# librosa/librosa

Hardware: AMD Instinct MI355X
Metric: STFT+mel frames/sec (n_fft=2048 hop=512) (higher is better)
Workload: dtype f32

## Files before the change

### librosa_amd/csrc/lra_kernels.h

```cpp
#pragma once

#ifndef LRA_ABLATE
#define LRA_ABLATE 0
#endif

#include <cmath>
#include <limits>

#include "lra_fft.h"

#if defined(LRA_PHASE_TIMER) && !defined(LRA_HOSTSIM)
__device__ unsigned long long lra_phase_ticks[16];
#define LRA_TICK(i)                                                    \
    do {                                                               \
        const unsigned long long now__ = __builtin_amdgcn_s_memtime(); \
        tick_acc[i] += now__ - tick_prev;                              \
        tick_prev = now__;                                             \
    } while (0)
#define LRA_TICK_DECL unsigned long long tick_acc[16] = {}, tick_prev = __builtin_amdgcn_s_memtime()
#define LRA_TICK_FLUSH                                                                    \
    do {                                                                                  \
        if ((threadIdx.x & 63) == 0)                                                      \
            for (int i__ = 0; i__ < 16; ++i__) atomicAdd(&lra_phase_ticks[i__], tick_acc[i__]); \
    } while (0)
// ... 676 lines not shown

template <class Cfg> LRA_HD void mel2_combine(const StftArgs<typename Cfg::real>& a, int clip, int frame, int tf, int it, int tile, Lds sh, Lds psum, Lds stage) {
    using T = typename Cfg::real;
    using C = typename Cfg::cplx;
    constexpr int NB = Cfg::M + 1;
#if LRA_ABLATE == 15
    if (a.n_mels != 12345) return;
#endif
    for (int m = tf; m < a.n_mels; m += Cfg::TF) {
        constexpr int UNR = 6;
        int first[2], cnt[2];
        LRA_UNROLL
        for (int h = 0; h < 2; ++h) {
            const int d = lds_ld<int>(sh, NB * (int)sizeof(C) + (Cfg::TF + m + h) * (int)sizeof(int));
            first[h] = d & 0xfff;
            cnt[h] = d >> 12;
        }
        T x[2][UNR];
        LRA_UNROLL
        for (int h = 0; h < 2; ++h) {
            LRA_UNROLL
            for (int q = 0; q < UNR; ++q) {
                const bool ok = q < cnt[h];
                x[h][q] = lds_ld<T>(psum, ((ok ? first[h] + q : 0) * 2 + (1 - h)) * (int)sizeof(T));
                if (!ok) x[h][q] = (T)0;
            }
        }
        T part[2];
        LRA_UNROLL
        for (int h = 0; h < 2; ++h) {
            T acc = (T)0;
            LRA_UNROLL
            for (int q = 0; q < UNR; ++q) acc += x[h][q];
            for (int q = UNR; q < cnt[h]; ++q) acc += lds_ld<T>(psum, ((first[h] + q) * 2 + (1 - h)) * (int)sizeof(T));
            part[h] = acc;
        }
        const T v = part[0] + part[1];
        if (tile == 1) a.Mel[((long long)clip * a.n_mels + m) * a.n_frames + frame] = v;
        else lds_st<T>(stage, (m * tile + (it % tile)) * (int)sizeof(T), v);
    }
}

constexpr int MELR_PMAX = 16;
template <class Cfg> LRA_HD int melr_w_slot(int i) { return i + 2 * (i / (Cfg::R / 2)); }
template <class Cfg> LRA_HD int melr_keep_off() { return ((melr_w_slot<Cfg>(Cfg::M) + 1) * 2 * (int)sizeof(typename Cfg::real) + 15) / 16 * 16; }
template <class Cfg> LRA_HD int melr_addr_off() { return melr_keep_off<Cfg>(); }
constexpr int MELR_PHOIST_N = 4;
template <class Cfg> LRA_HD bool melr_needs_table(int n_mels, int pmax) { return pmax > melr_ph<Cfg>() || n_mels > melr_nb<Cfg>() * Cfg::TF; }
template <class Cfg> LRA_HD int melr_shared_bytes(int n_mels, int pmax) {
    return ((melr_addr_off<Cfg>() + (melr_needs_table<Cfg>(n_mels, pmax) ? n_mels * 2 * pmax * (int)sizeof(int) : 0) + 15) / 16) * 16;
}
template <class Cfg> constexpr bool melr_fits() {
    return Cfg::R == 16 && (1 << Cfg::PADSHIFT) % (Cfg::R / 2) == 0 && (Cfg::R * Cfg::TF + 2) * 2 * (int)sizeof(typename Cfg::real) <= Cfg::FRAME_BYTES;
}

template <class Cfg> LRA_HD void melr_tables_to_lds(const StftArgs<typename Cfg::real>& a, int tid, Lds sh) {
    using T = typename Cfg::real;
    using C = typename Cfg::cplx;
    const C* __restrict__ w2 = reinterpret_cast<const C*>(a.melr_w);
    for (int k = tid; k < Cfg::M + 1; k += Cfg::NT) lds_st<C>(sh, melr_w_slot<Cfg>(k) * (int)sizeof(C), w2[k]);
    if (melr_needs_table<Cfg>(a.n_mels, a.melr_pmax))
        for (int i = tid; i < a.n_mels * 2 * a.melr_pmax; i += Cfg::NT) lds_st<int>(sh, melr_addr_off<Cfg>() + i * (int)sizeof(int), a.melr_addr[i]);
}

template <class Cfg> LRA_HD void split_read_runs(FftRegs<Cfg>& rg, Lds fr, int tf) {
    using C = typename Cfg::cplx;
    constexpr int BPL = Cfg::R / 2, M = Cfg::M;
    const int ba = Cfg::phys(BPL * tf) * (int)sizeof(C);
    const int bm = Cfg::phys(M - BPL * tf - 1) * (int)sizeof(C);
    const int b0 = Cfg::phys((M - BPL * tf) & (M - 1)) * (int)sizeof(C);
    LRA_UNROLL
    for (int j = 0; j < BPL; ++j) {
        rg.v[2 * j] = lds_ld<C>(fr, ba + j * (int)sizeof(C));
        rg.v[2 * j + 1] = lds_ld<C>(fr, j == 0 ? b0 : bm - (j - 1) * (int)sizeof(C));
    }
    if (tf == 0) rg.mid = lds_ld<C>(fr, Cfg::phys(M / 2) * (int)sizeof(C));
}

template <class Cfg, int PM> LRA_HD void melr_split_accumulate(const StftArgs<typename Cfg::real>& a, bool valid, int tf, FftRegs<Cfg>& rg, Lds rs, Lds sh) {
    using T = typename Cfg::real;
    using C = typename Cfg::cplx;
    constexpr int BPL = Cfg::R / 2, M = Cfg::M, TF = Cfg::TF;
    C ab[2 * BPL];
    LRA_UNROLL
    for (int j = 0; j < BPL; ++j) {
        const int k = BPL * tf + j;
        C xk, xm;
        if (k == 0) {
            const C z0 = rg.v[0];
            xk = mk<T>((T)2 * (z0.x + z0.y), (T)0);
            xm = mk<T>((T)2 * (z0.x - z0.y), (T)0);
            if (valid && a.nonfinite_flag && !(std::fabs(xk.x) <= std::numeric_limits<T>::max())) LRA_ATOMIC_OR(a.nonfinite_flag, 1u);
        } else {
            split_pair<T>(rg.v[2 * j], rg.v[2 * j + 1], Cfg::HOIST ? rg.twr[j] : a.twr[k], xk, xm);
        }
        const T pk = spec_power<T, PM>(xk, a.power), pm = spec_power<T, PM>(xm, a.power);
        const C wk = lds_ld<C>(sh, ((BPL + 2) * tf + j) * (int)sizeof(C)), wm = lds_ld<C>(sh, ((BPL + 2) * (TF + tf) + j) * (int)sizeof(C));
        ab[j] = mk<T>(wk.x * pk, wk.y * pk);
        ab[BPL + j] = mk<T>(wm.x * pm, wm.y * pm);
    }
    LRA_UNROLL
    for (int run = 0; run < 2; ++run) {
        C acc = mk<T>((T)0, (T)0);
        LRA_UNROLL
        for (int j = 0; j < BPL; ++j) {
            const int jj = run * BPL + j;
            const T keep = rg.keep[jj];
            acc = mk<T>(acc.x * keep + ab[jj].x, acc.y * keep + ab[jj].y);
            lds_st<C>(rs, (jj * TF + tf) * (int)sizeof(C), acc);
        }
    }
    if (tf == 0) {
        const C xmid = mk<T>((T)2 * rg.mid.x, (T)-2 * rg.mid.y);
        const T pmid = spec_power<T, PM>(xmid, a.power);
        const C wq = lds_ld<C>(sh, melr_w_slot<Cfg>(M) * (int)sizeof(C));
        lds_st<C>(rs, a.melr_mid, mk<T>(wq.x * pmid, wq.y * pmid));
        lds_st<C>(rs, a.melr_zero, mk<T>((T)0, (T)0));
    }
}

#ifndef LRA_MEL_PAIR_READS
#define LRA_MEL_PAIR_READS 1
#endif
template <class Cfg, class RG> LRA_HD void melr_hoist(const StftArgs<typename Cfg::real>& a, int tf, RG& rg, int base = 0) {
    constexpr int PH = RG::MELR_PHOIST;
    LRA_UNROLL
    for (int jj = 0; jj < Cfg::R; ++jj) rg.keep[jj] = a.melr_keep[jj * Cfg::TF + tf];
    LRA_UNROLL
    for (int b = 0; b < RG::MELR_NB; ++b) {
        const int m = RG::MELR_NB * tf + b;
        LRA_UNROLL
        for (int h = 0; h < 2; ++h) {
            LRA_UNROLL
            for (int q = 0; q < PH; ++q) {
                const int ad = base + (m < a.n_mels ? a.melr_addr[(h * a.melr_pmax + q) * a.n_mels + m] : a.melr_zero);
                rg.mad[b][h * PH + q] = (LRA_MEL_PAIR_READS && sizeof(typename Cfg::real) == 4) ? (ad & ~(2 * (int)sizeof(typename Cfg::real) - 1)) : ad;
            }
        }
    }
}

#ifndef LRA_MEL_ALIGNED_BURSTS
#define LRA_MEL_ALIGNED_BURSTS 1
#endif
#ifndef LRA_MEL_BURST16
#define LRA_MEL_BURST16 1
#endif
template <class Cfg, class RG> LRA_HD int melr_tile_slot(const StftArgs<typename Cfg::real>& a, int clip, int frame, int it, int b, long long row0) {
    constexpr int MT = RG::MELR_TILE;
    if (!LRA_MEL_ALIGNED_BURSTS) return it & (MT - 1);
    if ((a.n_frames & 3) == 0 && Cfg::TF >= 64) return (int)(((long long)clip * a.n_mels * a.n_frames + (long long)b * a.n_frames + frame) & (MT - 1));
    return (int)((row0 + frame) & (MT - 1));
}
template <class Cfg, class RG> LRA_HD void melr_burst(const StftArgs<typename Cfg::real>& a, long long row0, int frame, int s8, int it, int b, RG& rg) {
    using T = typename Cfg::real;
    constexpr int MT = RG::MELR_TILE;
    T* __restrict__ row = a.Mel + (row0 + frame - s8);
    if constexpr (sizeof(T) == 4 && (MT == 8 || MT == 4)) {
        if (LRA_MEL_BURST16 && s8 == MT - 1 && it >= MT - 1) {
            store4_unaligned(row, rg.mt[b][0], rg.mt[b][1], rg.mt[b][2], rg.mt[b][3]);
            if constexpr (MT == 8) store4_unaligned(row + 4, rg.mt[b][4], rg.mt[b][5], rg.mt[b][6], rg.mt[b][7]);
            return;
        }
    }
    LRA_UNROLL
    for (int k = 0; k < MT; ++k)
        if (k <= s8 && k >= s8 - it) row[k] = rg.mt[b][k];
}

template <class Cfg, class RG> LRA_HD void melr_combine(const StftArgs<typename Cfg::real>& a, int clip, int frame, int tf, int it, int tile, bool last_of_slot, RG& rg, Lds sh,
                                                        Lds rs, Lds stage, Lds rs_hoisted) {
    using T = typename Cfg::real;
    constexpr int PH = RG::MELR_PHOIST, TF = Cfg::TF, NB = RG::MELR_NB;
    const bool more = a.melr_pmax > PH;
    constexpr int GB = NB * 2 * PH > 16 ? 16 / (2 * PH) : NB;
    T x[NB][2 * PH];
    LRA_UNROLL
    for (int b = 0; b < NB; ++b) {
      if (b % GB == 0) {
        LRA_UNROLL
        for (int bb = b; bb < b + GB; ++bb) {
            LRA_UNROLL
            for (int q = 0; q < 2 * PH; ++q) {
                if constexpr (LRA_MEL_PAIR_READS && sizeof(T) == 4) {
                    const cx<T> pr = lds_ld<cx<T>>(rs_hoisted, rg.mad[bb][q]);
                    x[bb][q] = q < PH ? pr.y : pr.x;
                } else {
                    x[bb][q] = lds_ld<T>(rs_hoisted, rg.mad[bb][q]);
                }
            }
        }
      }
        const int m = NB * tf + b;
        if (m >= a.n_mels) break;
        T part[2];
        LRA_UNROLL
        for (int h = 0; h < 2; ++h) {
            T acc = (T)0;
            LRA_UNROLL
            for (int q = 0; q < PH; ++q) acc += x[b][h * PH + q];
            if (LRA_UNLIKELY(more)) {
                for (int q = PH; q < a.melr_pmax; ++q)
                    acc += lds_ld<T>(rs, lds_ld<int>(sh, melr_addr_off<Cfg>() + ((h * a.melr_pmax + q) * a.n_mels + m) * (int)sizeof(int)));
            }
            part[h] = acc;
        }
        const T v = part[0] + part[1];
        if (tile == 1) {
            constexpr int MT = RG::MELR_TILE;
            const long long row0 = ((long long)clip * a.n_mels + m) * a.n_frames;
            const int s8 = melr_tile_slot<Cfg, RG>(a, clip, frame, it, b, row0);
            LRA_UNROLL
            for (int k = 0; k < MT; ++k) rg.mt[b][k] = k == s8 ? v : rg.mt[b][k];
            if (last_of_slot || s8 == MT - 1) melr_burst<Cfg, RG>(a, row0, frame, s8, it, b, rg);
        } else {
            lds_st<T>(stage, (m * tile + (it % tile)) * (int)sizeof(T), v);
        }
    }
    for (int m = tf + NB * TF; m < a.n_mels; m += TF) {
        T part[2];
        LRA_UNROLL
        for (int h = 0; h < 2; ++h) {
            T acc = (T)0;
            for (int q = 0; q < a.melr_pmax; ++q)
                acc += lds_ld<T>(rs, lds_ld<int>(sh, melr_addr_off<Cfg>() + ((h * a.melr_pmax + q) * a.n_mels + m) * (int)sizeof(int)));
            part[h] = acc;
        }
        const T v = part[0] + part[1];
        if (tile == 1) a.Mel[((long long)clip * a.n_mels + m) * a.n_frames + frame] = v;
        else lds_st<T>(stage, (m * tile + (it % tile)) * (int)sizeof(T), v);
    }
}

#define LRA_MID_PASS(Cfg, p, rg, lds, tw, slot_bytes) LRA_MID_PASS_TO(Cfg, Cfg::P, p, rg, lds, tw, slot_bytes)
#define LRA_MID_PASS_TO(Cfg, END, p, rg, lds, tw, slot_bytes)                                             \
    if (END > p) {                                                                                        \
        LRA_PHASE(Cfg::NT, tid) {                                                                         \
            pass_read<Cfg, (p < Cfg::P ? p : 0)>(LRA_R(rg).v, lds_sub(lds, (slot_of<Cfg>(tid)) * (slot_bytes)), lane_of<Cfg>(tid)); \
        } LRA_PHASE_END_SYNC(Cfg::WAVE_SYNC)                                                              \
        LRA_TICK(2 * p);                                                                                  \
        LRA_PHASE(Cfg::NT, tid) {                                                                         \
            pass_dft<Cfg, (p < Cfg::P ? p : 0)>(LRA_R(rg), lane_of<Cfg>(tid), tw);                          \
            pass_write<Cfg, (p < Cfg::P ? p : 0)>(LRA_R(rg).v, lds_sub(lds, (slot_of<Cfg>(tid)) * (slot_bytes)), lane_of<Cfg>(tid)); \
        } LRA_PHASE_END_SYNC(Cfg::WAVE_SYNC)                                                              \
        LRA_TICK(2 * p + 1);                                                                              \
    }

template <class Cfg> constexpr int stft_ring_off() { return Cfg::FRAME_BYTES; }
template <class Cfg> constexpr int stft_tile_off() { return Cfg::FRAME_BYTES + Cfg::N * (int)sizeof(typename Cfg::real); }
template <class Cfg> inline int stft_slot_bytes(int mode, int n_mels, int tile) {
    int b = stft_tile_off<Cfg>();
    if (mode == OUT_MEL || ((mode == OUT_MEL2 || mode == OUT_MELR) && tile > 1)) b += ((n_mels * tile * (int)sizeof(typename Cfg::real) + 15) / 16) * 16;
    if (mode == OUT_MEL2) b += mel2_psum_bytes<Cfg>(n_mels);
    return b;
}

template <class Cfg, int MODE, int PM = POW_TWO, int RAM = 0> LRA_HD void stft_block(const StftArgs<typename Cfg::real>& a_in, const int blk, Lds lds) {
    constexpr bool RA = RAM == 1, DIRECT = RAM >= 2;
    constexpr int RHD = 1 << (RAM >= 3 ? RAM - 2 : 0);
    static_assert(RAM <= 2 || RegRing<Cfg, RHD>::ok, "register ring: the hop must be a whole number of pass-0 rows");
    static_assert(!DIRECT || MODE == OUT_COMPLEX || MODE == OUT_POWER, "direct framing serves the complex / power epilogues");
    StftArgs<typename Cfg::real> a = a_in;
    const int clip = blk / a.wg_per_clip;
    const int f_first = (blk % a.wg_per_clip) * a.frames_per_wg;
    const int iters = a.frames_per_wg / Cfg::FPB;
    const int slot_bytes = a.slot_bytes;
    const int tile = a.mel_tile;
    constexpr bool DEFER = MODE == OUT_MEL2 && !(LRA_ABLATE >= 11 && LRA_ABLATE <= 13);
#ifndef LRA_MEL_LATE_PF
#define LRA_MEL_LATE_PF 1
#endif
    constexpr bool LATE_PF = DEFER && LRA_MEL_LATE_PF;
#ifndef LRA_PF_EARLY
#define LRA_PF_EARLY 1
#endif
    constexpr bool PF_EARLY = !LATE_PF && LRA_PF_EARLY;
#ifndef LRA_SPLIT_ONE_BARRIER
#define LRA_SPLIT_ONE_BARRIER 1
#endif
    constexpr bool SPLIT_NO_LDS = LRA_SPLIT_ONE_BARRIER && (MODE == OUT_COMPLEX || MODE == OUT_POWER);
#ifndef LRA_MIRROR32
#define LRA_MIRROR32 1
#endif
    constexpr bool MIRROR = LRA_MIRROR32 && (RAM == 3 || RAM == 6 || LRA_MIRROR32 > 1) && mirror32_cfg_ok<Cfg>();
    constexpr int MID_END = Cfg::P - (MIRROR ? 1 : 0);
    LRA_REGS(FftRegs<Cfg>, rg, Cfg::NT);
    LRA_PHASE(Cfg::NT, tid) {
        hoist_tables<Cfg>(LRA_R(rg), lane_of<Cfg>(tid), a.win, a.tw, a.twr, false, MODE == OUT_MELR);
        if (MIRROR) mirror32_hoist<Cfg>(LRA_R(rg), lane_of<Cfg>(tid), a.tw, a.twr);
        if (MODE == OUT_MEL2) mel2_tables_to_lds<Cfg>(a, tid, lds_sub(lds, a.shared_off));
        if (MODE == OUT_MELR) {
            melr_tables_to_lds<Cfg>(a, tid, lds_sub(lds, a.shared_off));
            melr_hoist<Cfg>(a, lane_of<Cfg>(tid), LRA_R(rg));
        }
    } LRA_PHASE_END_SYNC(Cfg::WAVE_SYNC && MODE != OUT_MEL2 && MODE != OUT_MELR)
    LRA_PHASE(Cfg::NT, tid) {
        const int slot = slot_of<Cfg>(tid), tf = lane_of<Cfg>(tid);
        if (RHD > 1 || DIRECT) {
            LRA_UNROLL
            for (int e = 0; e < Cfg::R; ++e) LRA_R(rg).nxt[e] = mk<typename Cfg::real>((typename Cfg::real)0, (typename Cfg::real)0);
        }
        if (RHD > 1) {
            regring_fill<Cfg, RHD>(a, clip, f_first + slot * iters, tf, LRA_R(rg));
        } else if (DIRECT) {
            stft_direct_fetch<Cfg>(a, clip, f_first + slot * iters, tf, LRA_R(rg));
        } else {
            stft_ring_fill<Cfg>(a, clip, f_first + slot * iters, tf, lds_sub(lds, slot * slot_bytes + stft_ring_off<Cfg>()));
            if (PF_EARLY && iters > 1) stft_ring_prefetch<Cfg, RA>(a, clip, f_first + slot * iters + 1, tf, LRA_R(rg));
        }
    } LRA_PHASE_END_SYNC(Cfg::WAVE_SYNC)
    int done = 0;
    LRA_TICK_DECL;
    for (int it = 0; it < iters; ++it) {
        if (f_first + it >= a.n_frames) break;
        LRA_TICK(0);
        if (!Cfg::HOIST) { LRA_LAUNDER(a.win); LRA_LAUNDER(a.tw); LRA_LAUNDER(a.twr); }
        if (MODE == OUT_MELR) lra_setprio<LRA_V1_PRIO_A>();
        else if (MODE == OUT_COMPLEX || MODE == OUT_POWER) lra_setprio<LRA_V1_PRIO_CA>();
        LRA_PHASE(Cfg::NT, tid) {
            const int slot = slot_of<Cfg>(tid), tf = lane_of<Cfg>(tid), frame = f_first + slot * iters + it;
// ... 828 lines not shown
```

### librosa_amd/csrc/lra_kernels_pc.h

```cpp
#pragma once

#include "lra_kernels2.h"

namespace lra {

#ifndef LRA_PC_PRIO_PA
#define LRA_PC_PRIO_PA 3
#endif
#ifndef LRA_PC_PRIO_PS
#define LRA_PC_PRIO_PS 2
#endif
#ifndef LRA_PC_PRIO_CA
#define LRA_PC_PRIO_CA 0
#endif
#ifndef LRA_PC_PRIO_CB
#define LRA_PC_PRIO_CB 1
#endif
#ifndef LRA_PC_ROTATE
#define LRA_PC_ROTATE 1
#endif
#ifndef LRA_PC_SPIN_LIMIT
#define LRA_PC_SPIN_LIMIT (1 << 22)
#endif

template <class Cfg> struct PcLayout {
    using T = typename Cfg::real;
    static constexpr int NP = 2;
    static constexpr int NT = (NP + 1) * Cfg::TF;
    static constexpr int FRAME = Cfg::FRAME_BYTES;
    static constexpr int PW = (v2_pw_bytes<Cfg>() + 15) / 16 * 16;
    static constexpr int RS = ((Cfg::R * (Cfg::TF + LRA_MEL_RS_PITCH_EXTRA) + 2) * 2 * (int)sizeof(T) + 15) / 16 * 16;
    static constexpr int frame_off(int s) { return s * FRAME; }
    static constexpr int pw_off(int s) { return NP * FRAME + s * PW; }
    static constexpr int rs_off() { return NP * (FRAME + PW); }
    static constexpr int flags_off() { return rs_off() + RS; }
    static constexpr int ready_off(int s) { return flags_off() + 4 * s; }
    static constexpr int consumed_off(int s) { return flags_off() + 4 * (NP + s); }
    static constexpr int BYTES = flags_off() + 16;
};

template <class Cfg> constexpr bool pc_cfg_ok() { return v23_cfg_ok<Cfg>() && Cfg::TF == 64 && v2_pw_swz<Cfg>() && melr_fits<Cfg>() && sizeof(typename Cfg::real) == 4; }
template <class Cfg> LRA_HD bool pc_bank_ok(int n_mels, int pmax) { return n_mels >= 1 && n_mels <= 2 * Cfg::TF && pmax <= 4; }

template <class Cfg> LRA_HD bool pc_fits_budget(int hd, int power_mode) {
    if (power_mode != POW_TWO && power_mode != POW_ONE) return false;
    if (hd == 8) return true;
    return hd == 4 && (power_mode == POW_TWO || Cfg::PLAN == 1);
}

template <class Cfg> struct PcRegs {
    using T = typename Cfg::real;
    using C = typename Cfg::cplx;
    static constexpr int NB = 2, PH = 4, TILE = 8, NP = PcLayout<Cfg>::NP;
    C w[Cfg::R];
    C wq;
    T keep[Cfg::R];
    T pw[Cfg::R], pw_extra;
    int mad[NB][2 * PH];
    T mt[NP][NB][TILE];
};
template <class Cfg> struct PcTile {
    static constexpr int MELR_TILE = PcRegs<Cfg>::TILE;
    typename Cfg::real (&mt)[PcRegs<Cfg>::NB][PcRegs<Cfg>::TILE];
};

#ifdef LRA_HOSTSIM
LRA_HD int pc_flag_load(Lds l, int off) { return lds_ld<int>(l, off); }
LRA_HD void pc_flag_store(Lds l, int off, int v) { lds_st<int>(l, off, v); }
LRA_HD void pc_wait(Lds, int, int, unsigned int*) {}
LRA_HD void pc_fence() {}
#else
__device__ __forceinline__ void pc_fence() {
    __builtin_amdgcn_fence(__ATOMIC_RELEASE, "wavefront");
    __builtin_amdgcn_wave_barrier();
    __builtin_amdgcn_fence(__ATOMIC_ACQUIRE, "wavefront");
}
__device__ __forceinline__ int pc_flag_load(Lds l, int off) { return *(const volatile __attribute__((address_space(3))) int*)(l.base + off); }
__device__ __forceinline__ void pc_flag_store(Lds l, int off, int v) { *(volatile __attribute__((address_space(3))) int*)(l.base + off) = v; }
__device__ __forceinline__ void pc_wait(Lds l, int off, int want, unsigned int* sticky) {
    int spins = 0;
    while (true) {
        const int v = LRA_UNIFORM(pc_flag_load(l, off));
        if (LRA_LIKELY(v >= want)) break;
        if (LRA_UNLIKELY(++spins > LRA_PC_SPIN_LIMIT)) {
            if (sticky && (threadIdx.x & 63) == 0) atomicOr(sticky, 2u);
            break;
        }
        __builtin_amdgcn_s_sleep(2);
    }
    pc_fence();
}
#endif

template <class Cfg, int HD> LRA_HD void pc_producer_prologue(const StftArgs<typename Cfg::real>& a, int clip, int frame0, int tf, Regs2<Cfg, HD>& rg) {
    using T = typename Cfg::real;
    if constexpr (Cfg::PLAN == 1) v3_hoist<Cfg, HD>(rg, tf, a.win, a.tw, a.twr);
    else v2_hoist<Cfg, HD>(rg, tf, a.win, a.tw, a.twr);
    v2_fill<Cfg, HD>(a, clip, frame0, tf, rg);
    if constexpr (v2_rotate_asm_ok<Cfg, HD>() && LRA_PC_ROTATE) {
        LRA_UNROLL
        for (int e = 0; e < Cfg::R; ++e) { LRA_KEEP(rg.raw[e].x); LRA_KEEP(rg.raw[e].y); }
    }
    LRA_UNROLL
    for (int e = 0; e < Regs2<Cfg, HD>::NEW; ++e) rg.pf[e] = mk<T>((T)0, (T)0);
}
template <class Cfg, int HD> LRA_HD void pc_producer_pass0(const StftArgs<typename Cfg::real>& a, int clip, int frame, int it, bool more, int tf, Regs2<Cfg, HD>& rg, Lds fr) {
    if (v2_rotate_asm_ok<Cfg, HD>() && LRA_PC_ROTATE) {
        v2_window_rotating<Cfg, HD>(it, rg);
        if (more) v2_issue_loads<Cfg, HD>(a, clip, frame + 1, tf, rg);
        v2_pass0_dft<Cfg, HD>(tf, rg, fr);
    } else {
        if (it > 0) v2_shift<Cfg, HD>(rg);
        if (more) v2_issue_loads<Cfg, HD>(a, clip, frame + 1, tf, rg);
        v2_pass0<Cfg, HD>(frame < a.n_frames, tf, rg, fr);
    }
}

template <class Cfg, int p> LRA_HD void pc_mid_dft_write(typename Cfg::cplx* v, const typename Cfg::cplx* treg, Lds fr, int tf) {
    if constexpr (Cfg::PLAN == 1) {
        v3_mid_twiddle_dft<Cfg>(v, treg);
        v3_mid_write<Cfg>(v, fr, tf);
    } else {
        pass_twiddle_dft_reg<Cfg, p>(v, treg);
        pass_write<Cfg, p>(v, fr, tf);
    }
}
template <class Cfg, int HD> LRA_HD void pc_last_read(Regs2<Cfg, HD>& rg, Lds fr, int tf) {
    if constexpr (Cfg::PLAN == 1) v3_last_read<Cfg, HD>(rg, fr, tf);
    else v2_last_read<Cfg, HD>(rg, fr, tf);
}
template <class Cfg, int HD, int PM> LRA_HD void pc_last_power_row(const StftArgs<typename Cfg::real>& a, int clip, int frame, int tf, Regs2<Cfg, HD>& rg, Lds pwr) {
    if constexpr (Cfg::PLAN == 1) v3_last_split_store<Cfg, HD, OUT_MELR, PM, false>(a, clip, frame, frame < a.n_frames, tf, rg, pwr);
    else v2_last_split_store<Cfg, HD, OUT_MELR, PM, false, false>(a, clip, frame, frame < a.n_frames, tf, rg, pwr);
}

template <class Cfg> LRA_HD void pc_consumer_prologue(const StftArgs<typename Cfg::real>& a, int tf, PcRegs<Cfg>& rg) {
    using T = typename Cfg::real;
    using C = typename Cfg::cplx;
    using RG = PcRegs<Cfg>;
    constexpr int BPL = Cfg::R / 2, TF = Cfg::TF;
    const C* __restrict__ w2 = reinterpret_cast<const C*>(a.melr_w);
    LRA_UNROLL
    for (int run = 0; run < 2; ++run) {
        LRA_UNROLL
        for (int j = 0; j < BPL; ++j) rg.w[run * BPL + j] = w2[BPL * (run * TF + tf) + j];
    }
    rg.wq = w2[Cfg::M];
    LRA_UNROLL
    for (int jj = 0; jj < Cfg::R; ++jj) rg.keep[jj] = a.melr_keep[jj * TF + tf];
    LRA_UNROLL
    for (int b = 0; b < RG::NB; ++b) {
        const int m = RG::NB * tf + b;
        LRA_UNROLL
        for (int h = 0; h < 2; ++h) {
            LRA_UNROLL
            for (int q = 0; q < RG::PH; ++q) {
                const int ad = PcLayout<Cfg>::rs_off() + (m < a.n_mels ? a.melr_addr[(h * a.melr_pmax + q) * a.n_mels + m] : a.melr_zero);
                rg.mad[b][h * RG::PH + q] = ad & ~(2 * (int)sizeof(T) - 1);
            }
        }
    }
    LRA_UNROLL
    for (int s = 0; s < RG::NP; ++s) {
        LRA_UNROLL
        for (int b = 0; b < RG::NB; ++b) {
            LRA_UNROLL
            for (int k = 0; k < RG::TILE; ++k) rg.mt[s][b][k] = (T)0;
        }
    }
    rg.pw_extra = (T)0;
}
template <class Cfg> LRA_HD void pc_runs_read(PcRegs<Cfg>& rg, Lds pwr, int tf) {
    using T = typename Cfg::real;
    constexpr int BPL = Cfg::R / 2;
    static_assert(BPL == 8, "runs of 8 bins");
    LRA_UNROLL
    for (int run = 0; run < 2; ++run) {
        const int first = 8 * (run * Cfg::TF + tf);
        const V4<T> lo = lds_ld<V4<T>>(pwr, v2_pw_index<Cfg>(first) * (int)sizeof(T)), hi = lds_ld<V4<T>>(pwr, v2_pw_index<Cfg>(first + 4) * (int)sizeof(T));
        T* d = rg.pw + run * BPL;
        d[0] = lo.a; d[1] = lo.b; d[2] = lo.c; d[3] = lo.d; d[4] = hi.a; d[5] = hi.b; d[6] = hi.c; d[7] = hi.d;
    }
    rg.pw_extra = lds_ld<T>(pwr, (tf == 0 ? v2_pw_index<Cfg>(Cfg::M) : 0) * (int)sizeof(T));
}
template <class Cfg> LRA_HD void pc_accumulate(const StftArgs<typename Cfg::real>& a, int tf, PcRegs<Cfg>& rg, Lds rs) {
    using T = typename Cfg::real;
    using C = typename Cfg::cplx;
    constexpr int BPL = Cfg::R / 2, TF = Cfg::TF;
    LRA_UNROLL
    for (int run = 0; run < 2; ++run) {
        C acc = mk<T>((T)0, (T)0);
        LRA_UNROLL
        for (int j = 0; j < BPL; ++j) {
            const int jj = run * BPL + j;
            const T p = rg.pw[jj], keep = rg.keep[jj];
            acc = mk<T>(acc.x * keep + rg.w[jj].x * p, acc.y * keep + rg.w[jj].y * p);
            lds_st<C>(rs, (jj * mel_runs_pitch(TF, 1) + tf) * (int)sizeof(C), acc);
        }
    }
    if (tf == 0) {
        lds_st<C>(rs, a.melr_mid, mk<T>(rg.wq.x * rg.pw_extra, rg.wq.y * rg.pw_extra));
        lds_st<C>(rs, a.melr_zero, mk<T>((T)0, (T)0));
    }
}
template <class Cfg, int S> LRA_HD void pc_combine(const StftArgs<typename Cfg::real>& a, int clip, int frame, int tf, int it, bool last_of_slot, PcRegs<Cfg>& rg, Lds wg) {
    using T = typename Cfg::real;
    using RG = PcRegs<Cfg>;
    constexpr int PH = RG::PH, NB = RG::NB, MT = RG::TILE;
    T x[NB][2 * PH];
    LRA_UNROLL
    for (int b = 0; b < NB; ++b) {
        LRA_UNROLL
        for (int q = 0; q < 2 * PH; ++q) {
            const cx<T> pr = lds_ld<cx<T>>(wg, rg.mad[b][q]);
            x[b][q] = q < PH ? pr.y : pr.x;
        }
    }
    PcTile<Cfg> tile{rg.mt[S]};
    LRA_UNROLL
    for (int b = 0; b < NB; ++b) {
        const int m = NB * tf + b;
        if (m >= a.n_mels) break;
        T part[2];
        LRA_UNROLL
        for (int h = 0; h < 2; ++h) {
            T acc = (T)0;
            LRA_UNROLL
            for (int q = 0; q < PH; ++q) acc += x[b][h * PH + q];
            part[h] = acc;
        }
        const T v = part[0] + part[1];
        const long long row0 = ((long long)clip * a.n_mels + m) * a.n_frames;
        const int s8 = melr_tile_slot<Cfg, PcTile<Cfg>>(a, clip, frame, it, b, row0);
        LRA_UNROLL
        for (int k = 0; k < MT; ++k) rg.mt[S][b][k] = k == s8 ? v : rg.mt[S][b][k];
        if (last_of_slot || s8 == MT - 1) melr_burst<Cfg, PcTile<Cfg>>(a, row0, frame, s8, it, b, tile);
    }
}

template <class Cfg, int HD, int PM = POW_TWO> LRA_HD void stft_pc_block(const StftArgs<typename Cfg::real>& a_in, const int blk, Lds lds) {
    static_assert(pc_cfg_ok<Cfg>(), "producer / consumer mel kernel: one wave per frame, mirrored last pass, swizzled power row");
    using T = typename Cfg::real;
    using L = PcLayout<Cfg>;
    using RG = Regs2<Cfg, HD>;
    constexpr int NP = L::NP, TF = Cfg::TF;
    StftArgs<T> a = a_in;
    const int clip = blk / a.wg_per_clip;
    const int f_first = (blk % a.wg_per_clip) * a.frames_per_wg;
    const int iters = a.frames_per_wg / NP;
    const int left = a.n_frames - f_first;
    const int n_it = left < iters ? left : iters;
#ifdef LRA_HOSTSIM
    LRA_REGS(RG, prg, L::NT);
    LRA_REGS(PcRegs<Cfg>, crg, L::NT);
    LRA_PHASE(L::NT, tid) {
        const int w = tid / TF, tf = tid % TF;
        if (w < NP) pc_producer_prologue<Cfg, HD>(a, clip, f_first + w * iters, tf, LRA_R(prg));
        else pc_consumer_prologue<Cfg>(a, tf, LRA_R(crg));
        if (tid < 2 * NP) pc_flag_store(lds, L::flags_off() + 4 * tid, 0);
    } LRA_PHASE_END
    for (int it = 0; it < n_it; ++it) {
        LRA_PHASE(L::NT, tid) {
            const int w = tid / TF, tf = tid % TF;
            if (w < NP) pc_producer_pass0<Cfg, HD>(a, clip, f_first + w * iters + it, it, it + 1 < iters, tf, LRA_R(prg), lds_sub(lds, L::frame_off(w)));
        } LRA_PHASE_END_SYNC(true)
#define LRA_PC_MID(p)                                                                                                                   \
        if (Cfg::P - 1 > p) {                                                                                                           \
            LRA_PHASE(L::NT, tid) {                                                                                                     \
                if (tid / TF < NP) pass_read<Cfg, (p < Cfg::P ? p : 0)>(LRA_R(prg).v, lds_sub(lds, L::frame_off(tid / TF)), tid % TF);  \
            } LRA_PHASE_END_SYNC(true)                                                                                                  \
            LRA_PHASE(L::NT, tid) {                                                                                                     \
                if (tid / TF < NP) pc_mid_dft_write<Cfg, (p < Cfg::P ? p : 0)>(LRA_R(prg).v, LRA_R(prg).treg, lds_sub(lds, L::frame_off(tid / TF)), tid % TF); \
            } LRA_PHASE_END_SYNC(true)                                                                                                  \
        }
        LRA_PC_MID(1)
        LRA_PC_MID(2)
#undef LRA_PC_MID
        LRA_PHASE(L::NT, tid) {
            if (tid / TF < NP) pc_last_read<Cfg, HD>(LRA_R(prg), lds_sub(lds, L::frame_off(tid / TF)), tid % TF);
        } LRA_PHASE_END_SYNC(true)
        LRA_PHASE(L::NT, tid) {
            const int w = tid / TF, tf = tid % TF, frame = f_first + w * iters + it;
            if (w < NP) pc_last_power_row<Cfg, HD, PM>(a, clip, frame, tf, LRA_R(prg), lds_sub(lds, L::pw_off(w)));
        } LRA_PHASE_END
        for (int s = 0; s < NP; ++s) {
            LRA_PHASE(L::NT, tid) {
                if (tid / TF == NP) pc_runs_read<Cfg>(LRA_R(crg), lds_sub(lds, L::pw_off(s)), tid % TF);
            } LRA_PHASE_END_SYNC(true)
            LRA_PHASE(L::NT, tid) {
                if (tid / TF == NP) pc_accumulate<Cfg>(a, tid % TF, LRA_R(crg), lds_sub(lds, L::rs_off()));
            } LRA_PHASE_END_SYNC(true)
            LRA_PHASE(L::NT, tid) {
                const int tf = tid % TF, frame = f_first + s * iters + it;
                if (tid / TF == NP && frame < a.n_frames) {
                    const bool last = it + 1 == iters || frame + 1 >= a.n_frames;
                    if (s == 0) pc_combine<Cfg, 0>(a, clip, frame, tf, it, last, LRA_R(crg), lds);
                    else pc_combine<Cfg, 1>(a, clip, frame, tf, it, last, LRA_R(crg), lds);
                }
            } LRA_PHASE_END_SYNC(true)
        }
        sim::state().barrier();
    }
#else
    if (threadIdx.x < 2 * NP) pc_flag_store(lds, L::flags_off() + 4 * (int)threadIdx.x, 0);
    phase_sync<false>();
    const int wave = LRA_UNIFORM((int)(threadIdx.x / TF));
    if (wave < NP) {
        RG rg;
        const Lds fr = lds_sub(lds, L::frame_off(wave)), pwr = lds_sub(lds, L::pw_off(wave));
        {
            const int tf = phase_tid() % TF;
            pc_producer_prologue<Cfg, HD>(a, clip, f_first + wave * iters, tf, rg);
        }
        pc_fence();
        for (int it = 0; it < n_it; ++it) {
            const int frame = f_first + wave * iters + it;
            v2_setprio<LRA_PC_PRIO_PA>();
            {
                const int tf = phase_tid() % TF;
                pc_producer_pass0<Cfg, HD>(a, clip, frame, it, it + 1 < iters, tf, rg, fr);
            }
            pc_fence();
#define LRA_PC_MID(p)                                                                                    \
            if (Cfg::P - 1 > p) {                                                                        \
                { const int tf = phase_tid() % TF; pass_read<Cfg, (p < Cfg::P ? p : 0)>(rg.v, fr, tf); } \
                pc_fence();                                                                              \
                { const int tf = phase_tid() % TF; pc_mid_dft_write<Cfg, (p < Cfg::P ? p : 0)>(rg.v, rg.treg, fr, tf); } \
                pc_fence();                                                                              \
            }
            LRA_PC_MID(1)
            LRA_PC_MID(2)
#undef LRA_PC_MID
            int taken;
            {
                const int tf = phase_tid() % TF;
                pc_last_read<Cfg, HD>(rg, fr, tf);
                taken = pc_flag_load(lds, L::consumed_off(wave));
            }
            pc_fence();
            v2_setprio<LRA_PC_PRIO_PS>();
            if (LRA_UNLIKELY(LRA_UNIFORM(taken) < it)) pc_wait(lds, L::consumed_off(wave), it, a.nonfinite_flag);
            {
                const int tf = phase_tid() % TF;
                pc_last_power_row<Cfg, HD, PM>(a, clip, frame, tf, rg, pwr);
            }
            pc_fence();
            if (phase_tid() % TF == 0) pc_flag_store(lds, L::ready_off(wave), it + 1);
            pc_fence();
        }
    } else {
        PcRegs<Cfg> rg;
        const Lds rs = lds_sub(lds, L::rs_off());
        {
            const int tf = phase_tid() % TF;
            pc_consumer_prologue<Cfg>(a, tf, rg);
        }
        pc_fence();
        for (int it = 0; it < n_it; ++it) {
#define LRA_PC_SERVE(S)                                                                                                        \
            {                                                                                                                  \
                const int frame = f_first + S * iters + it;                                                                   \
                v2_setprio<LRA_PC_PRIO_CA>();                                                                                  \
                pc_wait(lds, L::ready_off(S), it + 1, a.nonfinite_flag);                                                                        \
                { const int tf = phase_tid() % TF; pc_runs_read<Cfg>(rg, lds_sub(lds, L::pw_off(S)), tf); }                    \
                pc_fence();                                                                                                    \
                if (phase_tid() % TF == 0) pc_flag_store(lds, L::consumed_off(S), it + 1);           \
                pc_fence();                                                                                                    \
                { const int tf = phase_tid() % TF; pc_accumulate<Cfg>(a, tf, rg, rs); }                                        \
                pc_fence();                                                                                                    \
                v2_setprio<LRA_PC_PRIO_CB>();                                                                                  \
                if (frame < a.n_frames) {                                                                                      \
                    const int tf = phase_tid() % TF;                                                                           \
                    pc_combine<Cfg, S>(a, clip, frame, tf, it, it + 1 == iters || frame + 1 >= a.n_frames, rg, lds);           \
                }                                                                                                              \
                pc_fence();                                                                                                    \
            }
            LRA_PC_SERVE(0)
            LRA_PC_SERVE(1)
#undef LRA_PC_SERVE
        }
    }
#endif
}

}
```

Measured before the change: 579.9 million.

## Streamline producer/consumer mel consumer: vector tile, hoisted addresses, uniform slot path

Reworks the consumer wave of the producer/consumer mel kernel. The per-band output tile becomes a 16-wide vector register value, and power-row LDS offsets, mel row pointers and per-slot phase offsets are precomputed in the prologue. A compile-time uniform-slot variant replaces the select-chain tile update with a direct indexed write, and LDS pair loads use precomputed raw addresses. A fast-path ready check skips the spin loop when the flag is already set. The aim is to cut integer address arithmetic and select instructions in the consumer's critical path, at the cost of more persistent registers and two template instantiations.

```diff
diff --git a/librosa_amd/csrc/lra_kernels.h b/librosa_amd/csrc/lra_kernels.h
--- a/librosa_amd/csrc/lra_kernels.h
+++ b/librosa_amd/csrc/lra_kernels.h
@@ -852,20 +852,20 @@
     if ((a.n_frames & 3) == 0 && Cfg::TF >= 64) return (int)(((long long)clip * a.n_mels * a.n_frames + (long long)b * a.n_frames + frame) & (MT - 1));
     return (int)((row0 + frame) & (MT - 1));
 }
-template <class Cfg, class RG> LRA_HD void melr_burst(const StftArgs<typename Cfg::real>& a, long long row0, int frame, int s8, int it, int b, RG& rg) {
-    using T = typename Cfg::real;
-    constexpr int MT = RG::MELR_TILE;
-    T* __restrict__ row = a.Mel + (row0 + frame - s8);
+template <class T, int MT> LRA_HD void melr_burst_row(T* __restrict__ row, int s8, int it, const T (&mt)[MT]) {
     if constexpr (sizeof(T) == 4 && (MT == 8 || MT == 4)) {
         if (LRA_MEL_BURST16 && s8 == MT - 1 && it >= MT - 1) {
-            store4_unaligned(row, rg.mt[b][0], rg.mt[b][1], rg.mt[b][2], rg.mt[b][3]);
-            if constexpr (MT == 8) store4_unaligned(row + 4, rg.mt[b][4], rg.mt[b][5], rg.mt[b][6], rg.mt[b][7]);
+            store4_unaligned(row, mt[0], mt[1], mt[2], mt[3]);
+            if constexpr (MT == 8) store4_unaligned(row + 4, mt[4], mt[5], mt[6], mt[7]);
             return;
         }
     }
     LRA_UNROLL
     for (int k = 0; k < MT; ++k)
-        if (k <= s8 && k >= s8 - it) row[k] = rg.mt[b][k];
+        if (k <= s8 && k >= s8 - it) row[k] = mt[k];
+}
+template <class Cfg, class RG> LRA_HD void melr_burst(const StftArgs<typename Cfg::real>& a, long long row0, int frame, int s8, int it, int b, RG& rg) {
+    melr_burst_row(a.Mel + (row0 + frame - s8), s8, it, rg.mt[b]);
 }
 
 template <class Cfg, class RG> LRA_HD void melr_combine(const StftArgs<typename Cfg::real>& a, int clip, int frame, int tf, int it, int tile, bool last_of_slot, RG& rg, Lds sh,
diff --git a/librosa_amd/csrc/lra_kernels_pc.h b/librosa_amd/csrc/lra_kernels_pc.h
--- a/librosa_amd/csrc/lra_kernels_pc.h
+++ b/librosa_amd/csrc/lra_kernels_pc.h
@@ -48,6 +48,16 @@
     return hd == 4 && (power_mode == POW_TWO || Cfg::PLAN == 1);
 }
 
+#ifdef LRA_HOSTSIM
+struct PcTileV {
+    float e[16];
+    float& operator[](int i) { return e[i]; }
+    float operator[](int i) const { return e[i]; }
+};
+#else
+typedef float PcTileV __attribute__((ext_vector_type(16)));
+#endif
+
 template <class Cfg> struct PcRegs {
     using T = typename Cfg::real;
     using C = typename Cfg::cplx;
@@ -57,12 +67,31 @@
     T keep[Cfg::R];
     T pw[Cfg::R], pw_extra;
     int mad[NB][2 * PH];
-    T mt[NP][NB][TILE];
+    int pwa[4], pwx;
+    T* row[NB];
+    int ph[NP][NB];
+    PcTileV mt[NP];
 };
-template <class Cfg> struct PcTile {
-    static constexpr int MELR_TILE = PcRegs<Cfg>::TILE;
-    typename Cfg::real (&mt)[PcRegs<Cfg>::NB][PcRegs<Cfg>::TILE];
-};
+template <class Cfg> LRA_HD bool pc_tile_uniform(const StftArgs<typename Cfg::real>& a) { return !LRA_MEL_ALIGNED_BURSTS || ((a.n_frames & 3) == 0 && Cfg::TF >= 64); }
+#ifdef LRA_HOSTSIM
+LRA_HD int pc_mad_addr(Lds wg, int ad) { return ad; }
+LRA_HD cx<float> pc_pair_ld(Lds wg, int addr) { return lds_ld<cx<float>>(wg, addr); }
+#else
+__device__ __forceinline__ int pc_mad_addr(Lds wg, int ad) {
+    int addr = (int)(unsigned int)(size_t)(__attribute__((address_space(3))) char*)(wg.base + ad);
+    asm volatile("" : "+v"(addr));
+    return addr;
+}
+__device__ __forceinline__ cx<float> pc_pair_ld(Lds, int addr) {
+    typedef float f2v __attribute__((ext_vector_type(2)));
+    const f2v t = *(const volatile __attribute__((address_space(3))) f2v*)(size_t)(unsigned int)addr;
+    return __builtin_bit_cast(cx<float>, t);
+}
+#endif
+template <class T, int MT> LRA_HD void pc_tile_band(const PcTileV& t, int b, T (&out)[MT]) {
+    LRA_UNROLL
+    for (int k = 0; k < MT; ++k) out[k] = t[MT * b + k];
+}
 
 #ifdef LRA_HOSTSIM
 LRA_HD int pc_flag_load(Lds l, int off) { return lds_ld<int>(l, off); }
@@ -90,6 +119,10 @@
     }
     pc_fence();
 }
+__device__ __forceinline__ void pc_wait_ready(Lds l, int off, int want, unsigned int* sticky) {
+    if (LRA_UNLIKELY(LRA_UNIFORM(pc_flag_load(l, off)) < want)) pc_wait(l, off, want, sticky);
+    else pc_fence();
+}
 #endif
 
 template <class Cfg, int HD> LRA_HD void pc_producer_prologue(const StftArgs<typename Cfg::real>& a, int clip, int frame0, int tf, Regs2<Cfg, HD>& rg) {
@@ -134,7 +167,7 @@
     else v2_last_split_store<Cfg, HD, OUT_MELR, PM, false, false>(a, clip, frame, frame < a.n_frames, tf, rg, pwr);
 }
 
-template <class Cfg> LRA_HD void pc_consumer_prologue(const StftArgs<typename Cfg::real>& a, int tf, PcRegs<Cfg>& rg) {
+template <class Cfg> LRA_HD void pc_consumer_prologue(const StftArgs<typename Cfg::real>& a, int clip, int f_first, int iters, int tf, PcRegs<Cfg>& rg, Lds wg) {
     using T = typename Cfg::real;
     using C = typename Cfg::cplx;
     using RG = PcRegs<Cfg>;
@@ -156,32 +189,44 @@
             LRA_UNROLL
             for (int q = 0; q < RG::PH; ++q) {
                 const int ad = PcLayout<Cfg>::rs_off() + (m < a.n_mels ? a.melr_addr[(h * a.melr_pmax + q) * a.n_mels + m] : a.melr_zero);
-                rg.mad[b][h * RG::PH + q] = ad & ~(2 * (int)sizeof(T) - 1);
+                rg.mad[b][h * RG::PH + q] = pc_mad_addr(wg, ad & ~(2 * (int)sizeof(T) - 1));
             }
         }
     }
     LRA_UNROLL
+    for (int run = 0; run < 2; ++run) {
+        const int first = 8 * (run * TF + tf);
+        rg.pwa[2 * run] = v2_pw_index<Cfg>(first) * (int)sizeof(T);
+        rg.pwa[2 * run + 1] = v2_pw_index<Cfg>(first + 4) * (int)sizeof(T);
+    }
+    rg.pwx = (tf == 0 ? v2_pw_index<Cfg>(Cfg::M) : 0) * (int)sizeof(T);
+    LRA_UNROLL
+    for (int b = 0; b < RG::NB; ++b) {
+        const int m = RG::NB * tf + b;
+        rg.row[b] = a.Mel + ((long long)clip * a.n_mels + (m < a.n_mels ? m : 0)) * a.n_frames;
+    }
+    LRA_UNROLL
     for (int s = 0; s < RG::NP; ++s) {
         LRA_UNROLL
         for (int b = 0; b < RG::NB; ++b) {
+            rg.ph[s][b] = LRA_MEL_ALIGNED_BURSTS ? (int)(((long long)clip * a.n_mels * a.n_frames + (long long)b * a.n_frames + f_first + s * iters) & (RG::TILE - 1)) : 0;
             LRA_UNROLL
-            for (int k = 0; k < RG::TILE; ++k) rg.mt[s][b][k] = (T)0;
+            for (int k = 0; k < RG::TILE; ++k) rg.mt[s][RG::TILE * b + k] = (T)0;
         }
     }
     rg.pw_extra = (T)0;
 }
-template <class Cfg> LRA_HD void pc_runs_read(PcRegs<Cfg>& rg, Lds pwr, int tf) {
+template <class Cfg> LRA_HD void pc_runs_read(PcRegs<Cfg>& rg, Lds pwr) {
     using T = typename Cfg::real;
     constexpr int BPL = Cfg::R / 2;
     static_assert(BPL == 8, "runs of 8 bins");
     LRA_UNROLL
     for (int run = 0; run < 2; ++run) {
-        const int first = 8 * (run * Cfg::TF + tf);
-        const V4<T> lo = lds_ld<V4<T>>(pwr, v2_pw_index<Cfg>(first) * (int)sizeof(T)), hi = lds_ld<V4<T>>(pwr, v2_pw_index<Cfg>(first + 4) * (int)sizeof(T));
+        const V4<T> lo = lds_ld<V4<T>>(pwr, rg.pwa[2 * run]), hi = lds_ld<V4<T>>(pwr, rg.pwa[2 * run + 1]);
         T* d = rg.pw + run * BPL;
         d[0] = lo.a; d[1] = lo.b; d[2] = lo.c; d[3] = lo.d; d[4] = hi.a; d[5] = hi.b; d[6] = hi.c; d[7] = hi.d;
     }
-    rg.pw_extra = lds_ld<T>(pwr, (tf == 0 ? v2_pw_index<Cfg>(Cfg::M) : 0) * (int)sizeof(T));
+    rg.pw_extra = lds_ld<T>(pwr, rg.pwx);
 }
 template <class Cfg> LRA_HD void pc_accumulate(const StftArgs<typename Cfg::real>& a, int tf, PcRegs<Cfg>& rg, Lds rs) {
     using T = typename Cfg::real;
@@ -203,7 +248,7 @@
         lds_st<C>(rs, a.melr_zero, mk<T>((T)0, (T)0));
     }
 }
-template <class Cfg, int S> LRA_HD void pc_combine(const StftArgs<typename Cfg::real>& a, int clip, int frame, int tf, int it, bool last_of_slot, PcRegs<Cfg>& rg, Lds wg) {
+template <class Cfg, int S, bool UNI> LRA_HD PcTileV pc_combine(const StftArgs<typename Cfg::real>& a, int clip, int frame, int tf, int it, bool last_of_slot, PcRegs<Cfg>& rg, Lds wg, PcTileV mt) {
     using T = typename Cfg::real;
     using RG = PcRegs<Cfg>;
     constexpr int PH = RG::PH, NB = RG::NB, MT = RG::TILE;
@@ -212,11 +257,10 @@
     for (int b = 0; b < NB; ++b) {
         LRA_UNROLL
         for (int q = 0; q < 2 * PH; ++q) {
-            const cx<T> pr = lds_ld<cx<T>>(wg, rg.mad[b][q]);
+            const cx<T> pr = pc_pair_ld(wg, rg.mad[b][q]);
             x[b][q] = q < PH ? pr.y : pr.x;
         }
     }
-    PcTile<Cfg> tile{rg.mt[S]};
     LRA_UNROLL
     for (int b = 0; b < NB; ++b) {
         const int m = NB * tf + b;
@@ -230,13 +274,55 @@
             part[h] = acc;
         }
         const T v = part[0] + part[1];
-        const long long row0 = ((long long)clip * a.n_mels + m) * a.n_frames;
-        const int s8 = melr_tile_slot<Cfg, PcTile<Cfg>>(a, clip, frame, it, b, row0);
-        LRA_UNROLL
-        for (int k = 0; k < MT; ++k) rg.mt[S][b][k] = k == s8 ? v : rg.mt[S][b][k];
-        if (last_of_slot || s8 == MT - 1) melr_burst<Cfg, PcTile<Cfg>>(a, row0, frame, s8, it, b, tile);
-    }
-}
+        int s8;
+        if constexpr (UNI) {
+            s8 = (rg.ph[S][b] + it) & (MT - 1);
+            mt[MT * b + s8] = v;
+        } else {
+            s8 = (int)((rg.row[b] - a.Mel + frame) & (MT - 1));
+            LRA_UNROLL
+            for (int k = 0; k < MT; ++k) mt[MT * b + k] = k == s8 ? v : mt[MT * b + k];
+        }
+        if (last_of_slot || s8 == MT - 1) {
+            T t8[MT];
+            pc_tile_band(mt, b, t8);
+            melr_burst_row(rg.row[b] + (frame - s8), s8, it, t8);
+        }
+    }
+    return mt;
+}
+
+#ifndef LRA_HOSTSIM
+template <class Cfg, bool UNI> __device__ __forceinline__ void pc_consumer(const StftArgs<typename Cfg::real>& a, int clip, int f_first, int iters, int n_it, Lds lds) {
+    using L = PcLayout<Cfg>;
+    constexpr int TF = Cfg::TF;
+    PcRegs<Cfg> rg;
+    const Lds rs = lds_sub(lds, L::rs_off());
+    const int tf = (int)(threadIdx.x & (TF - 1));
+    pc_consumer_prologue<Cfg>(a, clip, f_first, iters, tf, rg, lds);
+    pc_fence();
+    for (int it = 0; it < n_it; ++it) {
+#define LRA_PC_SERVE(S)                                                                                                        \
+        {                                                                                                                      \
+            const int frame = f_first + S * iters + it;                                                                       \
+            v2_setprio<LRA_PC_PRIO_CA>();                                                                                      \
+            pc_wait_ready(lds, L::ready_off(S), it + 1, a.nonfinite_flag);                                                     \
+            pc_runs_read<Cfg>(rg, lds_sub(lds, L::pw_off(S)));                                                                 \
+            pc_fence();                                                                                                        \
+            if (tf == 0) pc_flag_store(lds, L::consumed_off(S), it + 1);                             \
+            pc_fence();                                                                                                        \
+            pc_accumulate<Cfg>(a, tf, rg, rs);                                                                                 \
+            pc_fence();                                                                                                        \
+            v2_setprio<LRA_PC_PRIO_CB>();                                                                                      \
+            if (frame < a.n_frames) rg.mt[S] = pc_combine<Cfg, S, UNI>(a, clip, frame, tf, it, it + 1 == iters || frame + 1 >= a.n_frames, rg, lds, rg.mt[S]); \
+            pc_fence();                                                                                                        \
+        }
+        LRA_PC_SERVE(0)
+        LRA_PC_SERVE(1)
+#undef LRA_PC_SERVE
+    }
+}
+#endif
 
 template <class Cfg, int HD, int PM = POW_TWO> LRA_HD void stft_pc_block(const StftArgs<typename Cfg::real>& a_in, const int blk, Lds lds) {
     static_assert(pc_cfg_ok<Cfg>(), "producer / consumer mel kernel: one wave per frame, mirrored last pass, swizzled power row");
@@ -256,7 +342,7 @@
     LRA_PHASE(L::NT, tid) {
         const int w = tid / TF, tf = tid % TF;
         if (w < NP) pc_producer_prologue<Cfg, HD>(a, clip, f_first + w * iters, tf, LRA_R(prg));
-        else pc_consumer_prologue<Cfg>(a, tf, LRA_R(crg));
+        else pc_consumer_prologue<Cfg>(a, clip, f_first, iters, tf, LRA_R(crg), lds);
         if (tid < 2 * NP) pc_flag_store(lds, L::flags_off() + 4 * tid, 0);
     } LRA_PHASE_END
     for (int it = 0; it < n_it; ++it) {
@@ -285,7 +371,7 @@
         } LRA_PHASE_END
         for (int s = 0; s < NP; ++s) {
             LRA_PHASE(L::NT, tid) {
-                if (tid / TF == NP) pc_runs_read<Cfg>(LRA_R(crg), lds_sub(lds, L::pw_off(s)), tid % TF);
+                if (tid / TF == NP) pc_runs_read<Cfg>(LRA_R(crg), lds_sub(lds, L::pw_off(s)));
             } LRA_PHASE_END_SYNC(true)
             LRA_PHASE(L::NT, tid) {
                 if (tid / TF == NP) pc_accumulate<Cfg>(a, tid % TF, LRA_R(crg), lds_sub(lds, L::rs_off()));
@@ -294,8 +380,13 @@
                 const int tf = tid % TF, frame = f_first + s * iters + it;
                 if (tid / TF == NP && frame < a.n_frames) {
                     const bool last = it + 1 == iters || frame + 1 >= a.n_frames;
-                    if (s == 0) pc_combine<Cfg, 0>(a, clip, frame, tf, it, last, LRA_R(crg), lds);
-                    else pc_combine<Cfg, 1>(a, clip, frame, tf, it, last, LRA_R(crg), lds);
+                    if (pc_tile_uniform<Cfg>(a)) {
+                        if (s == 0) LRA_R(crg).mt[0] = pc_combine<Cfg, 0, true>(a, clip, frame, tf, it, last, LRA_R(crg), lds, LRA_R(crg).mt[0]);
+                        else LRA_R(crg).mt[1] = pc_combine<Cfg, 1, true>(a, clip, frame, tf, it, last, LRA_R(crg), lds, LRA_R(crg).mt[1]);
+                    } else {
+                        if (s == 0) LRA_R(crg).mt[0] = pc_combine<Cfg, 0, false>(a, clip, frame, tf, it, last, LRA_R(crg), lds, LRA_R(crg).mt[0]);
+                        else LRA_R(crg).mt[1] = pc_combine<Cfg, 1, false>(a, clip, frame, tf, it, last, LRA_R(crg), lds, LRA_R(crg).mt[1]);
+                    }
                 }
             } LRA_PHASE_END_SYNC(true)
         }
@@ -349,38 +440,10 @@
             pc_fence();
         }
     } else {
-        PcRegs<Cfg> rg;
-        const Lds rs = lds_sub(lds, L::rs_off());
-        {
-            const int tf = phase_tid() % TF;
-            pc_consumer_prologue<Cfg>(a, tf, rg);
-        }
-        pc_fence();
-        for (int it = 0; it < n_it; ++it) {
-#define LRA_PC_SERVE(S)                                                                                                        \
-            {                                                                                                                  \
-                const int frame = f_first + S * iters + it;                                                                   \
-                v2_setprio<LRA_PC_PRIO_CA>();                                                                                  \
-                pc_wait(lds, L::ready_off(S), it + 1, a.nonfinite_flag);                                                                        \
-                { const int tf = phase_tid() % TF; pc_runs_read<Cfg>(rg, lds_sub(lds, L::pw_off(S)), tf); }                    \
-                pc_fence();                                                                                                    \
-                if (phase_tid() % TF == 0) pc_flag_store(lds, L::consumed_off(S), it + 1);           \
-                pc_fence();                                                                                                    \
-                { const int tf = phase_tid() % TF; pc_accumulate<Cfg>(a, tf, rg, rs); }                                        \
-                pc_fence();                                                                                                    \
-                v2_setprio<LRA_PC_PRIO_CB>();                                                                                  \
-                if (frame < a.n_frames) {                                                                                      \
-                    const int tf = phase_tid() % TF;                                                                           \
-                    pc_combine<Cfg, S>(a, clip, frame, tf, it, it + 1 == iters || frame + 1 >= a.n_frames, rg, lds);           \
-                }                                                                                                              \
-                pc_fence();                                                                                                    \
-            }
-            LRA_PC_SERVE(0)
-            LRA_PC_SERVE(1)
-#undef LRA_PC_SERVE
-        }
-    }
-#endif
-}
-
-}
+        if (pc_tile_uniform<Cfg>(a)) pc_consumer<Cfg, true>(a, clip, f_first, iters, n_it, lds);
+        else pc_consumer<Cfg, false>(a, clip, f_first, iters, n_it, lds);
+    }
+#endif
+}
+
+}
```

Measured after the change: 621.5 million, median of 6. 7.2% higher.
